# liaochikon/SnowMocap

Measured on AMD Instinct MI355X. Metric: joint-triangulations/sec, higher is better.
Workload: dtype f64; 1 GPU; BASELINE configs[1]: 4 cameras x 1 person x 133 joints x 10000 frames per step per GPU, floor rig, default thresholds; steps cycle a pool of 32 distinct HBM-resident batches; cameras=4, persons=1, joints=133, method=pairwise (reference-exact), io=fp32 in / fp32 out, fp64 math, streams=2, context_overrides=, parallelism=frames sharded x1, no data-path collective

## Files before the change

snowmocap_amd/csrc/snowtri.hip:

```cpp
#include "../../include/snowtri.h"

#include <hip/hip_runtime.h>
#include <hip/hip_ext.h>

#include <algorithm>
#include <atomic>
#include <chrono>
#include <thread>
#include <cmath>
#include <cstdio>
#include <cstdlib>
#include <cstring>
#include <limits>
#include <map>
#include <mutex>
#include <new>
#include <string>
#include <vector>

#include "snowtri_fused.hpp"
#include "snowtri_lean.hpp"
#include "snowtri_cluster.hpp"
#include "snowtri_general.hpp"
#include "snowtri_assoc.hpp"
// ... 2437 lines not shown
    return SNOWTRI_OK;
}

constexpr int kLeanJ = 133;
constexpr int kFusedSingleMaxCams = 4;
constexpr int kLeanTilesPerWave = 4;

template <int C, typename TIn, typename TOut>
std::string lean_kernel_name(const char *kernel) {
    std::vector<std::string> args{std::to_string(C), type_name<TIn>(), std::to_string(kLeanJ)};
    if (sizeof(TOut) == 8) args.push_back("double");
    return kernel_name(kernel, args);
}

template <int C, typename TIn, typename TOut = float>
int launch_fused_lean(snowtri_ctx *ctx, hipStream_t st, int64_t F, const TIn *d_kpts, const int32_t *d_np,
                      const Params &prm, TOut *d_xyzs, TOut *d_ps, int32_t *d_cnt, uint32_t *d_fl) {
    constexpr int kScoreBytes = (int)sizeof(TOut);
    constexpr int NP = C * (C - 1) / 2;
    const int wg_small = ctx->lean_wg_per_cu, tpw = ctx->lean_tiles_per_wave > 0 ? ctx->lean_tiles_per_wave : kLeanTilesPerWave;
    const size_t per_block = general_scratch_bytes(NP, kLeanJ);
    auto kern = k_fused_lean<C, TIn, kLeanJ, TOut>;
    const int64_t W_small = (int64_t)ctx->num_cus * wg_small * kLeanWaves;
    const int64_t seg_max = (int64_t)kLeanTw * kLeanWaves * 512 * ((int64_t)ctx->num_cus * 6);
    LeanUnits<C, TOut> un{};
    if constexpr (LeanUnits<C, TOut>::kUsed) {
        un.lam = prm.dthr;
        un.inv = 1.0 / prm.dthr;
        un.kos = (0.00025 / (double)NP) / prm.dthr;
        for (int q = 0; q < NP; q++)
            for (int i = 0; i < 3; i++)
                un.d[3 * q + i] = (ctx->ht[3 * ctx->hpairs[2 * q + 1] + i] - ctx->ht[3 * ctx->hpairs[2 * q] + i]) * un.inv;
    }
    if (ctx->lean_coop != 0 && F <= (int64_t)ctx->num_cus * wg_small * kCoopMaxFrames) {
        const int grid = (int)std::min<int64_t>(F, (int64_t)ctx->num_cus * wg_small);
        const int base = (int)(F / grid);
        const int64_t rem = F % grid;
        const int nf_max = base + (rem ? 1 : 0);
        const size_t lds = lean_coop_lds_bytes(C, kLeanJ, nf_max, kScoreBytes);
        int rc = ctx->cur->work.ensure(per_block * (size_t)grid);
        if (rc) return rc;
        if (ctx->debug) fprintf(stderr, "k_fused_lean_coop: F %lld grid %d frames per tile %d (+1 for %lld) lds %zu\n", (long long)F, grid, base, (long long)rem, lds);
        rc = launch_kernel(ctx, st, k_fused_lean_coop<C, TIn, kLeanJ, TOut>, dim3(grid), dim3(kBlock), lds, true, F, base, rem, nf_max, ctx->rig(),
                           d_kpts, d_np, prm, un, d_xyzs, d_ps, d_cnt, d_fl, (char *)ctx->cur->work.p, per_block);
        if (rc) return rc;
        static const std::string cname = lean_kernel_name<C, TIn, TOut>("k_fused_lean_coop");
        ctx->last_kernels = cname.c_str();
        return SNOWTRI_OK;
    }
    if (ctx->timing && ctx->timing_attach && F > seg_max) {
        HIP_TRY(hipEventRecord(ctx->ev[0], st));
        HIP_TRY(hipEventRecord(ctx->ev_ring[2 * (ctx->ev_count % kTimingRing)], st));
    }
    for (int64_t s0 = 0; s0 < F; s0 += seg_max) {
        const int64_t Fs = std::min<int64_t>(seg_max, F - s0);
        int64_t W;
        if (Fs <= W_small * kLeanTw) {
            W = std::min<int64_t>(W_small, Fs);
        } else {
            const int64_t tiles0 = (Fs + kLeanTw - 1) / kLeanTw;
            W = std::max<int64_t>(W_small, (tiles0 + tpw - 1) / tpw);
        }
        const size_t scratch_mb = (size_t)ctx->lean_scratch_mb;
        const int64_t grid_cap = std::max<int64_t>((int64_t)ctx->num_cus * 6, (int64_t)((scratch_mb << 20) / per_block));
        const int grid = (int)std::min<int64_t>(grid_cap, (W + kLeanWaves - 1) / kLeanWaves);
        W = (int64_t)grid * kLeanWaves;
        const int64_t tiles_per_wave = (Fs + W * kLeanTw - 1) / (W * kLeanTw);
        const int64_t ntiles = std::min<int64_t>(Fs, W * tiles_per_wave);
// ... 13 lines not shown
            (void)hipOccupancyMaxActiveBlocksPerMultiprocessor(&occ, kern, kBlock, lds);
            fprintf(stderr, "k_fused_lean: F %lld grid %d tiles %lld (%d frames +1 for %lld) lds %zu occupancy/CU %d\n",
                    (long long)Fs, grid, (long long)ntiles, base, (long long)rem, lds, occ);
        }
    }
    static const std::string name = lean_kernel_name<C, TIn, TOut>("k_fused_lean");
    ctx->last_kernels = name.c_str();
    return SNOWTRI_OK;
}

template <typename TIn, typename TOut>
int launch_frame_general(snowtri_ctx *ctx, hipStream_t st, int64_t F, int Pmax, int J, const TIn *d_kpts,
                         const int32_t *d_np, const Params &prm, int Pout, TOut *d_xyzs, TOut *d_ps,
                         int32_t *d_cnt, uint32_t *d_fl) {
    const int64_t Kc = snowtri_num_candidate_slots(ctx->C, Pmax);
    if (Kc > kCondenseMaxN) return SNOWTRI_ERR_BAD_ARG;
    const size_t per_block = std::max<size_t>(256, general_scratch_bytes(Kc, J));
    int64_t grid = std::min<int64_t>(F, (int64_t)ctx->num_cus * 2);
    grid = std::max<int64_t>(1, std::min<int64_t>(grid, (int64_t)(kMaxScratchBytes / per_block)));
    int rc = ctx->cur->work.ensure(per_block * (size_t)grid);
    if (rc) return rc;
    rc = launch_kernel(ctx, st, k_frame_general<TIn, TOut>, dim3((int)grid), dim3(kBlock), condense_lds_bytes((int)Kc), false, F, Pmax, J, (int)Kc,
                       ctx->rig(), d_kpts, d_np, prm, Pout, d_xyzs, d_ps, d_cnt, d_fl, (char *)ctx->cur->work.p, per_block);
    if (rc) return rc;
    static const std::string name = kernel_name("k_frame_general", {type_name<TIn>(), type_name<TOut>()});
    ctx->last_kernels = name.c_str();
    return SNOWTRI_OK;
}

template <int C, typename TIn, typename TOut>
int launch_dlt_coop(snowtri_ctx *ctx, hipStream_t st, int64_t F, const TIn *d_kpts, const int32_t *d_np, const Params &prm, TOut *d_xyzs,
                    TOut *d_ps, int32_t *d_cnt, uint32_t *d_fl) {
    const int64_t resident = (int64_t)ctx->num_cus * kDltCoopWaves;
    const int64_t tiles = std::max<int64_t>((F + kCoopMaxFrames - 1) / kCoopMaxFrames, std::min<int64_t>(F, resident));
    const int base = (int)(F / tiles);
    const int64_t rem = F % tiles;
    const int nf_max = base + (rem ? 1 : 0);
    const size_t lds = dlt_coop_lds_bytes(C, kLeanJ, nf_max, (int)sizeof(TOut));
    int rc = launch_kernel(ctx, st, k_dlt_coop<C, TIn, kLeanJ, TOut>, dim3((unsigned)tiles), dim3(kBlock), lds, true, F, base, rem, nf_max,
                           ctx->rig(), d_kpts, d_np, prm, d_xyzs, d_ps, d_cnt, d_fl);
    if (rc) return rc;
    static const std::string name = kernel_name("k_dlt_coop", {std::to_string(C), type_name<TIn>(), std::to_string(kLeanJ), type_name<TOut>()});
    ctx->last_kernels = name.c_str();
    return SNOWTRI_OK;
}

struct SumsLaunch {
    int threads, lds, per_cu, Jc;
};
SumsLaunch sums_launch_shape(const snowtri_ctx *ctx, int Pmax, int J) {
    const int C = ctx->C, gs = p1_group_size(Pmax);
    const int64_t nitems = (int64_t)ctx->npairs * (Pmax / (gs >= 2 ? kSumsGA : 1)) * (Pmax / gs);
    SumsLaunch L;
    L.threads = ctx->sums_threads > 0 ? ctx->sums_threads : (nitems <= 256 ? 256 : (nitems <= 768 ? 512 : 1024));
    L.threads = L.threads <= 256 ? 256 : (L.threads <= 512 ? 512 : 1024);
    L.lds = ctx->sums_lds_kb > 0 ? ctx->sums_lds_kb * 1024 : (L.threads <= 256 ? 52 * 1024 : (L.threads <= 512 ? 80 * 1024 : 160 * 1024));
    L.lds = std::min(L.lds, 160 * 1024);
    L.per_cu = std::max(1, std::min((160 * 1024) / L.lds, 2048 / L.threads));
    const int pf = L.threads == 256 ? SumsShape<256>::kPrefetch : (L.threads == 512 ? SumsShape<512>::kPrefetch : SumsShape<1024>::kPrefetch);
    L.Jc = sums_chunk_joints(C, Pmax, J, ctx->npairs, L.threads, pf, L.lds);
    return L;
}

struct RecomputeRoute {
    bool can_hand, sumless, sums_kn, post_scores, stream, handover;
    bool split;
    SumsLaunch SL;
// ... 689 lines not shown
```

snowmocap_amd/csrc/snowtri_dlt_lean.hpp:

```cpp
#pragma once
#include "snowtri_lean.hpp"

namespace snowtri {

constexpr int kDltCoopWaves = 3;
__host__ __device__ constexpr size_t dlt_coop_lds_bytes(int C, int JC, int nf_max, int score_bytes = 4) {
    return (((size_t)96 * C + 8 * kDltFrame + (size_t)4 * (lean_coop_items_pad(JC, nf_max) + 128) + (size_t)score_bytes * lean_coop_items_pad(JC, nf_max) +
             (size_t)12 * kCoopMaxFrames + 16) + 15) & ~(size_t)15;
}

template <int C, typename TIn, int JC, typename TOut>
__global__ __launch_bounds__(kBlock, kDltCoopWaves) void k_dlt_coop(int64_t F, int tile_base, int64_t tile_rem, int nf_max, Rig rig,
                                                         const TIn *__restrict__ kpts, const int32_t *__restrict__ n_persons, Params prm,
                                                         TOut *__restrict__ out4, TOut *__restrict__ out_ps, int32_t *__restrict__ out_count,
                                                         uint32_t *__restrict__ out_flags) {
    extern __shared__ __attribute__((aligned(16))) char smem[];
    constexpr unsigned kRec = (unsigned)sizeof(Kp3<TIn>);
    constexpr unsigned kCamStride = (unsigned)JC * kRec;
    constexpr unsigned kOutRec = 4u * (unsigned)sizeof(TOut);
    const int tid = threadIdx.x, lane = tid & 63;
    const int wave = __builtin_amdgcn_readfirstlane(tid >> 6);
    const int items_pad = lean_coop_items_pad(JC, nf_max), ntable = items_pad + 128;
    double *Pl = reinterpret_cast<double *>(smem);
    uint32_t *table = reinterpret_cast<uint32_t *>(Pl + 12 * C + kDltFrame);
    TOut *stash = reinterpret_cast<TOut *>(table + ntable);
    double *favg = reinterpret_cast<double *>(stash + items_pad);
    uint32_t *fmask = reinterpret_cast<uint32_t *>(favg + kCoopMaxFrames);
    const Kp3<TIn> *kp3 = reinterpret_cast<const Kp3<TIn> *>(kpts);
    Kp3<TIn> bufA[C], bufB[C];

    int64_t f0;
    int nf;
    lean_tile_range((int64_t)blockIdx.x, tile_base, tile_rem, f0, nf);
    SNOWTRI_DEV_CHECK(f0 >= 0 && nf >= 1 && nf <= nf_max && nf_max <= kCoopMaxFrames && f0 + nf <= F, 34);
    const int npass_tile = (nf * JC + 63) >> 6;
    const int pos = (wave + 2 * (int)(blockIdx.x & 1u)) & (kLeanWaves - 1);
    const int pq = npass_tile / kLeanWaves, pr = npass_tile - pq * kLeanWaves;
    const int p0 = pos * pq + (pos < pr ? pos : pr), npass = pq + (pos < pr ? 1 : 0);
    const unsigned i0 = (unsigned)p0 * 64u;
    const __amdgpu_buffer_rsrc_t rin = lean_rsrc(kp3 + f0 * (int64_t)(C * JC), (unsigned)(nf * C * JC) * kRec);
    const __amdgpu_buffer_rsrc_t rout = lean_rsrc(reinterpret_cast<char *>(out4) + f0 * (int64_t)JC * kOutRec, (unsigned)(nf * JC) * kOutRec);
    auto fetch = [&](Kp3<TIn>(&dst)[C], unsigned voff) {
#pragma unroll
        for (int c = 0; c < C; c++)
            dst[c] = lean_load_kp3<TIn>(rin, voff + (unsigned)(c & 1) * kCamStride, (unsigned)(c & ~1) * kCamStride);
    };
    auto item_offset = [&](unsigned i) { return (i + (i / (unsigned)JC) * (unsigned)((C - 1) * JC)) * kRec; };
    const double cP = rig.P[tid < 12 * C + kDltFrame ? tid : 0];
    uint32_t cmask = 0xffffu;
    if (n_persons && tid < nf) {
        cmask = 0u;
        for (int c = 0; c < C; c++) cmask |= n_persons[(f0 + tid) * C + c] > 0 ? (1u << c) : 0u;
    }
    constexpr unsigned kNoItem = 0x40000000u;
    fetch(bufA, npass > 0 ? item_offset(i0 + (unsigned)lane) : kNoItem);
    for (unsigned i = (unsigned)tid; i < (unsigned)ntable; i += kBlock) table[i] = item_offset(i);
    if (tid < 12 * C + kDltFrame) Pl[tid] = cP;
    if (tid < kCoopMaxFrames) fmask[tid] = cmask;
    const bool masked = n_persons != nullptr;
    __syncthreads();

    auto solve_store = [&](const Kp3<TIn>(&buf)[C], unsigned out_off, TOut *stash_slot) {
        uint32_t m = 0xffffu;
        if (masked) {
            unsigned o = out_off;
            const unsigned fl = (o / kOutRec) / (unsigned)JC;
            m = fmask[fl < (unsigned)kCoopMaxFrames ? fl : 0u];
        }
        double x, y, z, os;
        asm volatile("" ::: "memory");
        dlt_item<C, TIn>(Pl, buf, m, prm, x, y, z, os);
        if constexpr (sizeof(TOut) == 4) {
            const float osf = (float)os;
            lean_u4 rec;
            rec.x = __float_as_uint((float)x);
            rec.y = __float_as_uint((float)y);
            rec.z = __float_as_uint((float)z);
            rec.w = __float_as_uint(osf);
            __builtin_amdgcn_raw_buffer_store_b128(rec, rout, (int)out_off, 0, kLeanStoreAux);
            *stash_slot = osf;
        } else {
            lean_u4 lo, hi;
            lo.x = (unsigned)__double2loint(x);
            lo.y = (unsigned)__double2hiint(x);
            lo.z = (unsigned)__double2loint(y);
            lo.w = (unsigned)__double2hiint(y);
            hi.x = (unsigned)__double2loint(z);
            hi.y = (unsigned)__double2hiint(z);
            hi.z = (unsigned)__double2loint(os);
            hi.w = (unsigned)__double2hiint(os);
            __builtin_amdgcn_raw_buffer_store_b128(lo, rout, (int)out_off, 0, kLeanStoreAux);
            __builtin_amdgcn_raw_buffer_store_b128(hi, rout, (int)out_off + 16, 0, kLeanStoreAux);
            *stash_slot = os;
        }
    };
    {
        unsigned out_off = (i0 + (unsigned)lane) * kOutRec;
        TOut *sp = stash + i0 + lane;
        const uint32_t *tp = table + i0 + lane;
        for (int k = 0; k < npass; k += 2) {
// ... 32 lines not shown
```

snowmocap_amd/csrc/snowtri_lean.hpp:

```cpp
#pragma once
#include "snowtri_fused.hpp"

namespace snowtri {

#ifndef SNOWTRI_LEAN_ROLLED_WAVES
#define SNOWTRI_LEAN_ROLLED_WAVES 2
#endif
#ifndef SNOWTRI_LEAN_ROLLED_RING
#define SNOWTRI_LEAN_ROLLED_RING 2
#endif
#ifndef SNOWTRI_LEAN_ROLLED_GROUP
#define SNOWTRI_LEAN_ROLLED_GROUP 4
#endif
constexpr int kLeanRolledWaves = SNOWTRI_LEAN_ROLLED_WAVES, kLeanRolledRing = SNOWTRI_LEAN_ROLLED_RING;
constexpr int kLeanRolledGroup = SNOWTRI_LEAN_ROLLED_GROUP;
#ifndef SNOWTRI_LEAN_AUTO_RESIDENT
#define SNOWTRI_LEAN_AUTO_RESIDENT 0
#endif
constexpr bool kLeanAutoResident = SNOWTRI_LEAN_AUTO_RESIDENT;
template <int C, typename TOut = float>
struct LeanShape {
    static constexpr bool kRolled = C >= 6 || (C == 5 && sizeof(TOut) == 8);
    static constexpr int kWaves = kRolled ? kLeanRolledWaves : kFastWaves;
    static constexpr int kRing = kRolled ? kLeanRolledRing : 3;
// ... 44 lines not shown
    if constexpr (sizeof(TIn) == 4) {
        const lean_u3 w = __builtin_amdgcn_raw_buffer_load_b96(r, (int)voff, (int)soff, kLeanLoadAux);
        k.u = __uint_as_float(w.x);
        k.v = __uint_as_float(w.y);
        k.s = __uint_as_float(w.z);
    } else {
        const lean_u4 w = __builtin_amdgcn_raw_buffer_load_b128(r, (int)voff, (int)soff, kLeanLoadAux);
        const lean_u2 z = __builtin_amdgcn_raw_buffer_load_b64(r, (int)voff + 16, (int)soff, kLeanLoadAux);
        k.u = __hiloint2double((int)w.y, (int)w.x);
        k.v = __hiloint2double((int)w.w, (int)w.z);
        k.s = __hiloint2double((int)z.y, (int)z.x);
    }
    return k;
}

__device__ __forceinline__ double uniform_f64(double x) {
    const int lo = __builtin_amdgcn_readfirstlane(__double2loint(x));
    const int hi = __builtin_amdgcn_readfirstlane(__double2hiint(x));
    return __hiloint2double(hi, lo);
}

__device__ __forceinline__ double uniform_lane_f64(double x, int lane) {
    const int lo = __builtin_amdgcn_readlane(__double2loint(x), lane);
    const int hi = __builtin_amdgcn_readlane(__double2hiint(x), lane);
    return __hiloint2double(hi, lo);
}

__device__ __forceinline__ float select_by_mask(float x, unsigned long long mask) {
    float r;
    asm("v_cndmask_b32_e64 %0, 0, %1, %2" : "=v"(r) : "v"(x), "s"(mask));
    return r;
}

template <int NK>
__device__ __forceinline__ void lean_rig_regs_load(double (&Kr)[NK], const double *__restrict__ Mlds) {
    constexpr int C = NK / 12;
#pragma unroll
    for (int i = 0; i < 9 * C + 3; i++) Kr[i] = Mlds[i];
#pragma unroll
    for (int i = 9 * C + 3; i < NK; i++) Kr[i] = Mlds[lean_scaled_at(C) + i - (9 * C + 3)];
#pragma unroll
    for (int i = 0; i < NK; i++) asm volatile("" : "+v"(Kr[i]));
}

template <int C, bool kResident, typename TIn, int NK>
__device__ __forceinline__ bool lean_item(const double *__restrict__ Mlds, const double (&Kr)[NK],
                                          const double (&dS)[3 * (C * (C - 1) / 2)],
                                          const Kp3<TIn> (&cur)[C], float kthr_f32, double kthr, double lam, double kos,
                                          float &ox, float &oy, float &oz, double &os) {
#pragma clang fp contract(off)
    double Mp[9 * C];
    const double *tp;
    if constexpr (kResident) {
        static_assert(NK == 12 * C, "Kr: M[C][9], t_0, t'[1 .. C-1][3]");
#pragma unroll
        for (int i = 0; i < 9 * C; i++) Mp[i] = Kr[i];
        tp = Kr + 9 * C;
    } else {
#pragma unroll
        for (int i = 0; i < 9 * C; i++) Mp[i] = Mlds[i];
        __builtin_amdgcn_sched_barrier(0);
        tp = Mlds + 9 * C;
    }
    double tq[3 * C];
#pragma unroll
    for (int i = 3; i < 3 * C; i++) {
        if constexpr (kResident)
            tq[i] = Kr[9 * C + i];
        else
            tq[i] = dS[i - 3];
    }
    Vec3 h[C], X[C];
    double a[C], alpha[C], beta[C];
    unsigned long long okm[C];
#pragma unroll
    for (int c = 0; c < C; c++) {
        const double u = (double)cur[c].u, v = (double)cur[c].v;
        h[c].x = fma(Mp[9 * c + 0], u, fma(Mp[9 * c + 1], v, Mp[9 * c + 2]));
        h[c].y = fma(Mp[9 * c + 3], u, fma(Mp[9 * c + 4], v, Mp[9 * c + 5]));
        h[c].z = fma(Mp[9 * c + 6], u, fma(Mp[9 * c + 7], v, Mp[9 * c + 8]));
        a[c] = dot3(h[c], h[c]);
        if constexpr (sizeof(TIn) == 4)
            okm[c] = __ballot(!((float)cur[c].s < kthr_f32));
        else
            okm[c] = __ballot(!((double)cur[c].s < kthr));
        if (c >= 1) {
            X[c].x = fma(h[c].y, tq[3 * c + 2], -(h[c].z * tq[3 * c + 1]));
            X[c].y = fma(h[c].z, tq[3 * c + 0], -(h[c].x * tq[3 * c + 2]));
            X[c].z = fma(h[c].x, tq[3 * c + 1], -(h[c].y * tq[3 * c + 0]));
        }
    }
    int q = 0;
#pragma unroll
    for (int mc = 0; mc < C - 1; mc++) {
#pragma unroll
        for (int sc = mc + 1; sc < C; sc++, q++) {
            const Vec3 &hm = h[mc], &hs = h[sc];
            const double dx = mc == 0 ? tq[3 * sc] : dS[3 * q], dy = mc == 0 ? tq[3 * sc + 1] : dS[3 * q + 1],
                         dz = mc == 0 ? tq[3 * sc + 2] : dS[3 * q + 2];
            const double b = dot3(hm, hs);
            const double det = a[mc] * a[sc] - b * b;
            const double e = fma(hm.z, dz, fma(hm.y, dy, hm.x * dx));
            const double g = fma(hs.z, dz, fma(hs.y, dy, hs.x * dx));
// ... 190 lines not shown
    const double cD = rig.pairc[tid < 3 * NP ? 6 * (tid / 3) + tid % 3 : 0];
    const int32_t cP = rig.pairs[tid < 2 * NP ? tid : 0];
    double dS[kRolled ? 1 : 3 * NP];
    constexpr bool kResident = !kRolled && kLeanAutoResident;
    double Kr[kResident ? 12 * C : 1];
    if constexpr (!kRolled) {
#pragma unroll
        for (int i = 0; i < 3 * NP; i++) dS[i] = un.d[i];
    }
    int64_t tile = (int64_t)blockIdx.x * kLeanWaves + wave;
    int64_t f0 = 0;
    int nf = 0;
    if (tile < ntiles) {
        lean_tile_range(tile, tile_base, tile_rem, f0, nf);
        const __amdgpu_buffer_rsrc_t rin = lean_rsrc(kp3 + f0 * (int64_t)(C * JC), (unsigned)(nf * C * JC) * kRec);
        fetch(bufA, rin, voff0);
        if constexpr (kRing >= 3) fetch(bufB, rin, voff1);
    }
    for (unsigned i = (unsigned)tid; i < (unsigned)kTable; i += kBlock)
        table[i] = (i + (i / (unsigned)JC) * (unsigned)((C - 1) * JC)) * kRec;
    for (int i = tid; i < slow_words; i += kBlock) slowbits[i] = 0u;
    if (tid < 9 * C) Mlds[tid] = cM;
    if (tid < 3 * C) Mlds[9 * C + tid] = cT;
    if (tid < 3 * NP) Mlds[12 * C + tid] = cD;
    if constexpr (!kRolled) {
        if (tid < 3 * NP) Mlds[lean_scaled_at(C) + tid] = cD * un.inv;
    }
    int32_t *pairs_lds = reinterpret_cast<int32_t *>(Mlds + 12 * C + 3 * NP);
    if (tid < 2 * NP) pairs_lds[tid] = cP;
    const float kthr_f32 = prm.kthr_f32;
    const double kthr = prm.kthr, dthr2 = prm.dthr2;
    const double ctol2_lo = prm.ctol < 0.0 ? -1.0 : prm.ctol * prm.ctol * (1.0 - 1e-12);
    __syncthreads();
    if constexpr (kResident) lean_rig_regs_load(Kr, Mlds);

    for (int ord = 0; tile < ntiles; tile += wstride, ord++) {
        SNOWTRI_DEV_CHECK(f0 >= 0 && nf >= 1 && nf <= kLeanTw && f0 + nf <= F, 1);
        SNOWTRI_DEV_CHECK((ord * kLeanWaves + wave + 1) << kLeanSlowShift <= slow_words * 32, 2);
        const __amdgpu_buffer_rsrc_t rin = lean_rsrc(kp3 + f0 * (int64_t)(C * JC), (unsigned)(nf * C * JC) * kRec);
        const __amdgpu_buffer_rsrc_t rout =
            lean_rsrc(reinterpret_cast<char *>(out4) + f0 * (int64_t)JC * kOutRec, (unsigned)(nf * JC) * kOutRec);
        const unsigned last = (unsigned)(nf * JC - 1);
        const int npass = (nf * JC + 63) >> 6;
        const unsigned slow_base = (unsigned)((ord * kLeanWaves + wave) << kLeanSlowShift);
        constexpr int kCheckFrames = 64 / NP;
        constexpr int kCheckPre = kRolled ? 0 : 2;
        Kp3<TIn> ckm[kCheckPre ? kCheckPre : 1], cks[kCheckPre ? kCheckPre : 1];
#pragma unroll
        for (int pass = 0; pass < kCheckPre; pass++) {
            const int wl = lane / NP, qq = lane - wl * NP, w = pass * kCheckFrames + wl;
            const bool live = wl < kCheckFrames && w < nf;
            const Kp3<TIn> *p = kp3 + (f0 + (live ? w : 0)) * (int64_t)(C * JC) + prm.center;
            ckm[pass] = p[pairs_lds[2 * qq] * JC];
            cks[pass] = p[pairs_lds[2 * qq + 1] * JC];
        }

        auto solve_store = [&](const Kp3<TIn>(&buf)[C], unsigned out_off, TOut *stash_slot) {
            const bool bad = lean_solve_store<C, kResident, TIn, TOut>(Mlds, Kr, dS, buf, kthr_f32, kthr, dthr2, un.lam, un.kos, rout, out_off, stash_slot);
            if (__ballot(bad)) {
                unsigned o = out_off;
                asm volatile("" : "+v"(o));
                const unsigned i = o / kOutRec;
                const unsigned bit = slow_base + i / (unsigned)JC;
                if (bad && i <= last) atomicOr(&slowbits[bit >> 5], 1u << (bit & 31u));
            }
        };
        unsigned out_off = (unsigned)lane * kOutRec;
// ... 54 lines not shown
                km = ckm[pass];
                ks = cks[pass];
            } else {
                const Kp3<TIn> *p = kp3 + (f0_cur + (live ? w : 0)) * (int64_t)(C * JC) + prm.center;
                km = p[mc * JC];
                ks = p[sc * JC];
            }
            const bool far = lean_centre_far<C, TIn>(Mlds, mc, sc, qq, lane, km, ks, ctol2_lo);
            if (live && far) {
                const unsigned bit = slow_base + (unsigned)w;
                atomicOr(&slowbits[bit >> 5], 1u << (bit & 31u));
            }
        }
        __builtin_amdgcn_fence(__ATOMIC_ACQ_REL, "wavefront");
        {
            constexpr int G = 4;
            const int w = lane / G, sub = lane & (G - 1);
            const bool live = w < nf_cur;
            const int64_t f = f0_cur + (live ? w : 0);
            double sum = 0.0;
            if (live) sum = lean_row_partial<JC, TOut>(stash + w * JC, sub);
            int not_one = 0;
            if (n_persons && live)
                for (int c = sub; c < C; c += G) not_one |= n_persons[f * C + c] != 1;
#pragma unroll
            for (int off = G / 2; off > 0; off >>= 1) {
                sum += __shfl_xor(sum, off, 64);
                not_one |= __shfl_xor(not_one, off, 64);
            }
            if (live && sub == 0) {
                const double avg = sum / (double)JC;
                const unsigned bit = slow_base + (unsigned)w;
                const bool slow = ((slowbits[bit >> 5] >> (bit & 31u)) & 1u) != 0u || !(avg >= prm.score_tol) ||
                                  fabs(avg - prm.score_tol) < 1e-6 * fabs(prm.score_tol) || not_one != 0;
                if (slow) {
                    atomicOr(&slowbits[bit >> 5], 1u << (bit & 31u));
                } else {
                    out_count[f] = 1;
                    if (out_ps) out_ps[f] = (TOut)avg;
                    if (out_flags) out_flags[f] = kFlagFast;
                }
            }
        }
        __builtin_amdgcn_fence(__ATOMIC_ACQ_REL, "wavefront");
    }

    __syncthreads();
    unsigned any = 0u;
    for (int i = lane; i < slow_words; i += 64) any |= slowbits[i];
    if (__ballot(any != 0u) == 0ull) return;
    {
        const PackedWriter<TOut> wr{out4, out_ps};
        double *slab = reinterpret_cast<double *>(scratch + (size_t)blockIdx.x * scratch_per_block);
        for (int wd = 0; wd < slow_words; wd++) {
            uint32_t m = slowbits[wd];
            __syncthreads();
            while (m) {
                const int bpos = __ffs((int)m) - 1;
                m &= m - 1u;
                const unsigned bit = (unsigned)(wd * 32 + bpos);
                const unsigned slot = bit >> kLeanSlowShift;
                const int64_t t = (int64_t)blockIdx.x * kLeanWaves + (slot % kLeanWaves) + (int64_t)(slot / kLeanWaves) * wstride;
                int64_t tf0;
                int tnf;
                lean_tile_range(t, tile_base, tile_rem, tf0, tnf);
                general_frame<TIn>(tf0 + (bit & ((1u << kLeanSlowShift) - 1u)), 1, JC, NP, rig, kpts, n_persons, prm, 1, wr,
                                   out_count, out_flags, slab, smem);
            }
        }
    }
}

constexpr int kCoopMaxFrames = 32;
__host__ __device__ constexpr int lean_coop_items_pad(int JC, int nf_max) { return (nf_max * JC + 63) / 64 * 64; }
__host__ __device__ constexpr size_t lean_coop_lds_bytes(int C, int JC, int nf_max, int score_bytes = 4) {
    return (((size_t)8 * lean_const_doubles(C) + (size_t)score_bytes * lean_coop_items_pad(JC, nf_max) + (size_t)8 * kCoopMaxFrames + 16) + 15) & ~(size_t)15;
}

template <int C, typename TIn, int JC, typename TOut = float>
__global__ __launch_bounds__(kBlock, (LeanShape<C, TOut>::kWaves)) void k_fused_lean_coop(
    int64_t F, int tile_base, int64_t tile_rem, int nf_max, Rig rig, const TIn *__restrict__ kpts, const int32_t *__restrict__ n_persons,
    Params prm, LeanUnits<C, TOut> un, TOut *__restrict__ out4, TOut *__restrict__ out_ps, int32_t *__restrict__ out_count,
    uint32_t *__restrict__ out_flags, char *scratch, size_t scratch_per_block) {
    extern __shared__ __attribute__((aligned(16))) char smem[];
    constexpr int NP = C * (C - 1) / 2;
    constexpr int kConstDoubles = lean_const_doubles(C);
    constexpr unsigned kRec = (unsigned)sizeof(Kp3<TIn>);
    constexpr unsigned kCamStride = (unsigned)JC * kRec;
    const int tid = threadIdx.x, lane = tid & 63;
    const int wave = __builtin_amdgcn_readfirstlane(tid >> 6);
    const int items_pad = lean_coop_items_pad(JC, nf_max);
    double *Mlds = reinterpret_cast<double *>(smem);
    TOut *stash = reinterpret_cast<TOut *>(Mlds + kConstDoubles);
    double *favg = reinterpret_cast<double *>(stash + items_pad);
    uint32_t *slowbits = reinterpret_cast<uint32_t *>(favg + kCoopMaxFrames);
    const Kp3<TIn> *kp3 = reinterpret_cast<const Kp3<TIn> *>(kpts);
    constexpr bool kRolled = LeanShape<C, TOut>::kRolled;
    constexpr unsigned kOutRec = 4u * (unsigned)sizeof(TOut);
    static_assert(sizeof(TOut) == 4 || kRolled, "float64 outputs: the rolled item only");
    constexpr int kRing = (kRolled && sizeof(TIn) == 8 && C >= 8) ? 1 : LeanShape<C, TOut>::kRing;
    Kp3<TIn> bufA[C], bufB[kRing >= 2 ? C : 1], bufC[kRing >= 3 ? C : 1];

#ifdef SNOWTRI_LEAN_TRACE
    unsigned long long *trace = reinterpret_cast<unsigned long long *>(scratch + (size_t)blockIdx.x * scratch_per_block) + 8 * (threadIdx.x >> 6);
#define SNOWTRI_STAMP(i) do { if ((threadIdx.x & 63) == 0) trace[i] = __builtin_amdgcn_s_memrealtime(); } while (0)
#else
#define SNOWTRI_STAMP(i) ((void)0)
#endif
    SNOWTRI_STAMP(0);
#ifdef SNOWTRI_LEAN_TRACE
    if ((threadIdx.x & 63) == 0) {
        unsigned hw, xcc;
        asm volatile("s_getreg_b32 %0, hwreg(HW_REG_HW_ID)" : "=s"(hw));
        asm volatile("s_getreg_b32 %0, hwreg(HW_REG_XCC_ID)" : "=s"(xcc));
        trace[7] = ((unsigned long long)xcc << 32) | hw;
    }
#endif
    int64_t f0;
    int nf;
    lean_tile_range((int64_t)blockIdx.x, tile_base, tile_rem, f0, nf);
    SNOWTRI_DEV_CHECK(f0 >= 0 && nf >= 1 && nf <= nf_max && nf_max <= kCoopMaxFrames && f0 + nf <= F, 3);
    const int npass_tile = (nf * JC + 63) >> 6;
    const int pos = (wave + 2 * (int)(blockIdx.x & 1u)) & (kLeanWaves - 1);
    const int pq = npass_tile / kLeanWaves, pr = npass_tile - pq * kLeanWaves;
    const int p0 = pos * pq + (pos < pr ? pos : pr), npass = pq + (pos < pr ? 1 : 0);
    const unsigned i0 = (unsigned)p0 * 64u;
    const __amdgpu_buffer_rsrc_t rin = lean_rsrc(kp3 + f0 * (int64_t)(C * JC), (unsigned)(nf * C * JC) * kRec);
    const __amdgpu_buffer_rsrc_t rout = lean_rsrc(reinterpret_cast<char *>(out4) + f0 * (int64_t)JC * kOutRec, (unsigned)(nf * JC) * kOutRec);
    const unsigned last = (unsigned)(nf * JC - 1);
    auto fetch = [&](Kp3<TIn>(&dst)[C], unsigned voff) {
#pragma unroll
        for (int c = 0; c < C; c++)
            dst[c] = lean_load_kp3<TIn>(rin, voff + (unsigned)(c & 1) * kCamStride, (unsigned)(c & ~1) * kCamStride);
    };
    static_assert(JC > 64, "one frame boundary per pass of 64 joints");
    constexpr unsigned kNoItem = 0x40000000u;
    constexpr unsigned kFrameSkip = (unsigned)((C - 1) * JC) * kRec;
    unsigned sj = i0 % (unsigned)JC, sbase = (i0 + (i0 / (unsigned)JC) * (unsigned)((C - 1) * JC)) * kRec;
    const unsigned lane_off = (unsigned)lane * kRec;
    auto next_offset = [&](bool own) {
        const unsigned o = lane_off + (own ? sbase : kNoItem) + ((unsigned)lane >= (unsigned)JC - sj ? kFrameSkip : 0u);
        sj += 64u;
        sbase += 64u * kRec;
        if (sj >= (unsigned)JC) {
            sj -= (unsigned)JC;
            sbase += kFrameSkip;
        }
        return o;
    };
    const double cM = rig.M[tid < 9 * C ? tid : 0], cT = rig.t[tid < 3 * C ? tid : 0];
    const double cD = rig.pairc[tid < 3 * NP ? 6 * (tid / 3) + tid % 3 : 0];
    const int32_t cP = rig.pairs[tid < 2 * NP ? tid : 0];
    double dS[kRolled ? 1 : 3 * NP];
    constexpr bool kResident = !kRolled && C == 4 && sizeof(TIn) == 4;
    double Kr[kResident ? 12 * C : 1];
    if constexpr (!kRolled) {
#pragma unroll
        for (int i = 0; i < 3 * NP; i++) dS[i] = un.d[i];
    }
    fetch(bufA, next_offset(npass > 0));
    if constexpr (kRing >= 3) fetch(bufB, next_offset(npass > 1));
    constexpr int kCheckFrames = 64 / NP;
    const int ncheck = (nf + kCheckFrames - 1) / kCheckFrames;
    Kp3<TIn> ckm, cks;
    int32_t *pairs_lds = reinterpret_cast<int32_t *>(Mlds + 12 * C + 3 * NP);
    if (tid == 0) slowbits[0] = 0u;
    if (tid < 9 * C) Mlds[tid] = cM;
    if (tid < 3 * C) Mlds[9 * C + tid] = cT;
    if (tid < 3 * NP) Mlds[12 * C + tid] = cD;
    if constexpr (!kRolled) {
        if (tid < 3 * NP) Mlds[lean_scaled_at(C) + tid] = cD * un.inv;
    }
    if (tid < 2 * NP) pairs_lds[tid] = cP;
    const float kthr_f32 = prm.kthr_f32;
    const double kthr = prm.kthr, dthr2 = prm.dthr2;
    const double ctol2_lo = prm.ctol < 0.0 ? -1.0 : prm.ctol * prm.ctol * (1.0 - 1e-12);
    SNOWTRI_STAMP(1);
    __syncthreads();
    SNOWTRI_STAMP(2);
    if constexpr (kResident) lean_rig_regs_load(Kr, Mlds);
    {
        const int wl = lane / NP, qq = lane - wl * NP, w = pos * kCheckFrames + wl;
        const bool live = pos < ncheck && wl < kCheckFrames && w < nf;
        const Kp3<TIn> *p = kp3 + (f0 + (live ? w : 0)) * (int64_t)(C * JC) + prm.center;
        ckm = p[pairs_lds[2 * qq] * JC];
        cks = p[pairs_lds[2 * qq + 1] * JC];
    }

    auto solve_store = [&](const Kp3<TIn>(&buf)[C], unsigned out_off, TOut *stash_slot) {
        const bool bad = lean_solve_store<C, kResident, TIn, TOut>(Mlds, Kr, dS, buf, kthr_f32, kthr, dthr2, un.lam, un.kos, rout, out_off, stash_slot);
        if (__ballot(bad)) {
            unsigned o = out_off;
            asm volatile("" : "+v"(o));
            const unsigned i = o / kOutRec;
            if (bad && i <= last) atomicOr(&slowbits[0], 1u << (i / (unsigned)JC));
        }
    };
    {
        unsigned out_off = (i0 + (unsigned)lane) * kOutRec;
        TOut *sp = stash + i0 + lane;
        if constexpr (kRing >= 3) {
            for (int k = 0; k < npass; k += 3) {
                fetch(bufC, next_offset(k + 2 < npass));
                solve_store(bufA, out_off, sp);
                fetch(bufA, next_offset(k + 3 < npass));
                if (k + 1 < npass) solve_store(bufB, out_off + 64u * kOutRec, sp + 64);
                fetch(bufB, next_offset(k + 4 < npass));
                if (k + 2 < npass) solve_store(bufC, out_off + 128u * kOutRec, sp + 128);
                out_off += 192u * kOutRec;
                sp += 192;
            }
        } else if constexpr (kRing == 2) {
            for (int k = 0; k < npass; k += 2) {
                fetch(bufB, next_offset(k + 1 < npass));
                solve_store(bufA, out_off, sp);
                fetch(bufA, next_offset(k + 2 < npass));
                if (k + 1 < npass) solve_store(bufB, out_off + 64u * kOutRec, sp + 64);
                out_off += 128u * kOutRec;
                sp += 128;
            }
        } else {
            for (int k = 0; k < npass; k++) {
                solve_store(bufA, out_off, sp);
                fetch(bufA, next_offset(k + 1 < npass));
                out_off += 64u * kOutRec;
                sp += 64;
            }
        }
    }
    SNOWTRI_STAMP(3);
    __syncthreads();
    SNOWTRI_STAMP(4);

    for (int pass = pos; pass < ncheck; pass += kLeanWaves) {
        const int wl = lane / NP, qq = lane - wl * NP, w = pass * kCheckFrames + wl;
        const bool live = wl < kCheckFrames && w < nf;
        const int mc = pairs_lds[2 * qq], sc = pairs_lds[2 * qq + 1];
        Kp3<TIn> km = ckm, ks = cks;
        if (pass != pos) {
            const Kp3<TIn> *p = kp3 + (f0 + (live ? w : 0)) * (int64_t)(C * JC) + prm.center;
            km = p[mc * JC];
            ks = p[sc * JC];
        }
        const bool far = lean_centre_far<C, TIn>(Mlds, mc, sc, qq, lane, km, ks, ctol2_lo);
        if (live && far) atomicOr(&slowbits[0], 1u << w);
    }
    {
        constexpr int G = 4;
        const int nmean = (nf + 64 / G - 1) / (64 / G);
        for (int pass = (pos - ncheck) & (kLeanWaves - 1); pass < nmean; pass += kLeanWaves) {
            const int w = pass * (64 / G) + lane / G, sub = lane & (G - 1);
            const bool live = w < nf;
            const int64_t f = f0 + (live ? w : 0);
            double sum = 0.0;
            if (live) sum = lean_row_partial<JC, TOut>(stash + w * JC, sub);
            int not_one = 0;
            if (n_persons && live)
                for (int c = sub; c < C; c += G) not_one |= n_persons[f * C + c] != 1;
#pragma unroll
            for (int off = G / 2; off > 0; off >>= 1) {
                sum += __shfl_xor(sum, off, 64);
                not_one |= __shfl_xor(not_one, off, 64);
            }
            if (live && sub == 0) {
                const double avg = sum / (double)JC;
                favg[w] = avg;
                if (!(avg >= prm.score_tol) || fabs(avg - prm.score_tol) < 1e-6 * fabs(prm.score_tol) || not_one != 0)
                    atomicOr(&slowbits[0], 1u << w);
            }
        }
    }
    SNOWTRI_STAMP(5);
    __syncthreads();
    const uint32_t slow = slowbits[0];
    if (wave == 0 && lane < nf && !((slow >> lane) & 1u)) {
        const int64_t f = f0 + lane;
        out_count[f] = 1;
        if (out_ps) out_ps[f] = (TOut)favg[lane];
        if (out_flags) out_flags[f] = kFlagFast;
    }
    SNOWTRI_STAMP(6);
    if (slow == 0u) return;
    {
        const PackedWriter<TOut> wr{out4, out_ps};
        double *slab = reinterpret_cast<double *>(scratch + (size_t)blockIdx.x * scratch_per_block);
        uint32_t m = slow;
        __syncthreads();
        while (m) {
            const int bpos = __ffs((int)m) - 1;
            m &= m - 1u;
            general_frame<TIn>(f0 + bpos, 1, JC, NP, rig, kpts, n_persons, prm, 1, wr, out_count, out_flags, slab, smem);
        }
    }
}

}
```

Measured before the change: 69.03 billion joints/s.

## Widen coop lean tiles, scalarize input streaming, and drop per-item bad checks

Splits the coop frame limit into a 64-frame cap, used only with an off-by-default overlap mode, and a 32-frame lone cap, with slow-frame bitmasks widened to 64 bits. Adds compile-time trims that are on by default: a scalar-offset buffer resource per fetch to cut per-lane address math, keeping only t_0 resident in registers instead of all translations, and skipping the per-item ballot/atomic for bad solves in the resident path. To keep fallbacks correct without the per-item check, the frame-level test now also marks non-finite score sums as slow. The DLT coop kernel gets its own 32-frame constant. These trims aim to cut VGPR pressure and instruction count in the hot loop, at the cost of relying on the score-sum check to catch bad items.

```diff
diff --git a/snowmocap_amd/csrc/snowtri.hip b/snowmocap_amd/csrc/snowtri.hip
--- a/snowmocap_amd/csrc/snowtri.hip
+++ b/snowmocap_amd/csrc/snowtri.hip
@@ -2493,8 +2493,10 @@
             for (int i = 0; i < 3; i++)
                 un.d[3 * q + i] = (ctx->ht[3 * ctx->hpairs[2 * q + 1] + i] - ctx->ht[3 * ctx->hpairs[2 * q] + i]) * un.inv;
     }
-    if (ctx->lean_coop != 0 && F <= (int64_t)ctx->num_cus * wg_small * kCoopMaxFrames) {
-        const int grid = (int)std::min<int64_t>(F, (int64_t)ctx->num_cus * wg_small);
+    const bool beside = kCoopOverlapWide && ctx->overlap >= 2 && ctx->cur != &ctx->sets[0] && F <= (int64_t)ctx->num_cus * kCoopMaxFrames;
+    const int wg_coop = beside ? 1 : wg_small;
+    if (ctx->lean_coop != 0 && F <= (int64_t)ctx->num_cus * wg_coop * (beside ? kCoopMaxFrames : kCoopLoneFrames)) {
+        const int grid = (int)std::min<int64_t>(F, (int64_t)ctx->num_cus * wg_coop);
         const int base = (int)(F / grid);
         const int64_t rem = F % grid;
         const int nf_max = base + (rem ? 1 : 0);
@@ -2574,7 +2576,7 @@
 int launch_dlt_coop(snowtri_ctx *ctx, hipStream_t st, int64_t F, const TIn *d_kpts, const int32_t *d_np, const Params &prm, TOut *d_xyzs,
                     TOut *d_ps, int32_t *d_cnt, uint32_t *d_fl) {
     const int64_t resident = (int64_t)ctx->num_cus * kDltCoopWaves;
-    const int64_t tiles = std::max<int64_t>((F + kCoopMaxFrames - 1) / kCoopMaxFrames, std::min<int64_t>(F, resident));
+    const int64_t tiles = std::max<int64_t>((F + kDltCoopMaxFrames - 1) / kDltCoopMaxFrames, std::min<int64_t>(F, resident));
     const int base = (int)(F / tiles);
     const int64_t rem = F % tiles;
     const int nf_max = base + (rem ? 1 : 0);
diff --git a/snowmocap_amd/csrc/snowtri_dlt_lean.hpp b/snowmocap_amd/csrc/snowtri_dlt_lean.hpp
--- a/snowmocap_amd/csrc/snowtri_dlt_lean.hpp
+++ b/snowmocap_amd/csrc/snowtri_dlt_lean.hpp
@@ -3,10 +3,11 @@
 
 namespace snowtri {
 
+constexpr int kDltCoopMaxFrames = 32;
 constexpr int kDltCoopWaves = 3;
 __host__ __device__ constexpr size_t dlt_coop_lds_bytes(int C, int JC, int nf_max, int score_bytes = 4) {
     return (((size_t)96 * C + 8 * kDltFrame + (size_t)4 * (lean_coop_items_pad(JC, nf_max) + 128) + (size_t)score_bytes * lean_coop_items_pad(JC, nf_max) +
-             (size_t)12 * kCoopMaxFrames + 16) + 15) & ~(size_t)15;
+             (size_t)12 * kDltCoopMaxFrames + 16) + 15) & ~(size_t)15;
 }
 
 template <int C, typename TIn, int JC, typename TOut>
@@ -25,14 +26,14 @@
     uint32_t *table = reinterpret_cast<uint32_t *>(Pl + 12 * C + kDltFrame);
     TOut *stash = reinterpret_cast<TOut *>(table + ntable);
     double *favg = reinterpret_cast<double *>(stash + items_pad);
-    uint32_t *fmask = reinterpret_cast<uint32_t *>(favg + kCoopMaxFrames);
+    uint32_t *fmask = reinterpret_cast<uint32_t *>(favg + kDltCoopMaxFrames);
     const Kp3<TIn> *kp3 = reinterpret_cast<const Kp3<TIn> *>(kpts);
     Kp3<TIn> bufA[C], bufB[C];
 
     int64_t f0;
     int nf;
     lean_tile_range((int64_t)blockIdx.x, tile_base, tile_rem, f0, nf);
-    SNOWTRI_DEV_CHECK(f0 >= 0 && nf >= 1 && nf <= nf_max && nf_max <= kCoopMaxFrames && f0 + nf <= F, 34);
+    SNOWTRI_DEV_CHECK(f0 >= 0 && nf >= 1 && nf <= nf_max && nf_max <= kDltCoopMaxFrames && f0 + nf <= F, 34);
     const int npass_tile = (nf * JC + 63) >> 6;
     const int pos = (wave + 2 * (int)(blockIdx.x & 1u)) & (kLeanWaves - 1);
     const int pq = npass_tile / kLeanWaves, pr = npass_tile - pq * kLeanWaves;
@@ -56,7 +57,7 @@
     fetch(bufA, npass > 0 ? item_offset(i0 + (unsigned)lane) : kNoItem);
     for (unsigned i = (unsigned)tid; i < (unsigned)ntable; i += kBlock) table[i] = item_offset(i);
     if (tid < 12 * C + kDltFrame) Pl[tid] = cP;
-    if (tid < kCoopMaxFrames) fmask[tid] = cmask;
+    if (tid < kDltCoopMaxFrames) fmask[tid] = cmask;
     const bool masked = n_persons != nullptr;
     __syncthreads();
 
@@ -65,7 +66,7 @@
         if (masked) {
             unsigned o = out_off;
             const unsigned fl = (o / kOutRec) / (unsigned)JC;
-            m = fmask[fl < (unsigned)kCoopMaxFrames ? fl : 0u];
+            m = fmask[fl < (unsigned)kDltCoopMaxFrames ? fl : 0u];
         }
         double x, y, z, os;
         asm volatile("" ::: "memory");
diff --git a/snowmocap_amd/csrc/snowtri_lean.hpp b/snowmocap_amd/csrc/snowtri_lean.hpp
--- a/snowmocap_amd/csrc/snowtri_lean.hpp
+++ b/snowmocap_amd/csrc/snowtri_lean.hpp
@@ -100,9 +100,9 @@
     return r;
 }
 
-template <int NK>
+template <int C, int NK>
 __device__ __forceinline__ void lean_rig_regs_load(double (&Kr)[NK], const double *__restrict__ Mlds) {
-    constexpr int C = NK / 12;
+    static_assert(NK == 12 * C || NK == 9 * C + 3, "Kr: M[C][9], t_0 and, at 12 C, t'[1 .. C-1][3]");
 #pragma unroll
     for (int i = 0; i < 9 * C + 3; i++) Kr[i] = Mlds[i];
 #pragma unroll
@@ -119,8 +119,9 @@
 #pragma clang fp contract(off)
     double Mp[9 * C];
     const double *tp;
+    constexpr bool kScalarT = !kResident || NK == 9 * C + 3;
     if constexpr (kResident) {
-        static_assert(NK == 12 * C, "Kr: M[C][9], t_0, t'[1 .. C-1][3]");
+        static_assert(NK == 12 * C || NK == 9 * C + 3, "Kr: M[C][9], t_0 and, at 12 C, t'[1 .. C-1][3]");
 #pragma unroll
         for (int i = 0; i < 9 * C; i++) Mp[i] = Kr[i];
         tp = Kr + 9 * C;
@@ -133,10 +134,10 @@
     double tq[3 * C];
 #pragma unroll
     for (int i = 3; i < 3 * C; i++) {
-        if constexpr (kResident)
+        if constexpr (kScalarT)
+            tq[i] = dS[i - 3];
+        else
             tq[i] = Kr[9 * C + i];
-        else
-            tq[i] = dS[i - 3];
     }
     Vec3 h[C], X[C];
     double a[C], alpha[C], beta[C];
@@ -393,7 +394,7 @@
     const double kthr = prm.kthr, dthr2 = prm.dthr2;
     const double ctol2_lo = prm.ctol < 0.0 ? -1.0 : prm.ctol * prm.ctol * (1.0 - 1e-12);
     __syncthreads();
-    if constexpr (kResident) lean_rig_regs_load(Kr, Mlds);
+    if constexpr (kResident) lean_rig_regs_load<C>(Kr, Mlds);
 
     for (int ord = 0; tile < ntiles; tile += wstride, ord++) {
         SNOWTRI_DEV_CHECK(f0 >= 0 && nf >= 1 && nf <= kLeanTw && f0 + nf <= F, 1);
@@ -514,7 +515,8 @@
                 const double avg = sum / (double)JC;
                 const unsigned bit = slow_base + (unsigned)w;
                 const bool slow = ((slowbits[bit >> 5] >> (bit & 31u)) & 1u) != 0u || !(avg >= prm.score_tol) ||
-                                  fabs(avg - prm.score_tol) < 1e-6 * fabs(prm.score_tol) || not_one != 0;
+                                  fabs(avg - prm.score_tol) < 1e-6 * fabs(prm.score_tol) || not_one != 0 ||
+                                  !(fabs(sum) < INFINITY);
                 if (slow) {
                     atomicOr(&slowbits[bit >> 5], 1u << (bit & 31u));
                 } else {
@@ -553,7 +555,17 @@
     }
 }
 
-constexpr int kCoopMaxFrames = 32;
+constexpr int kCoopMaxFrames = 64;
+constexpr int kCoopLoneFrames = 32;
+#ifndef SNOWTRI_COOP_OVERLAP_WIDE
+#define SNOWTRI_COOP_OVERLAP_WIDE 0
+#endif
+constexpr bool kCoopOverlapWide = SNOWTRI_COOP_OVERLAP_WIDE;
+#ifndef SNOWTRI_COOP_TRIMS
+#define SNOWTRI_COOP_TRIMS 7
+#endif
+constexpr bool kCoopNoItemCheck = (SNOWTRI_COOP_TRIMS & 1) != 0, kCoopScalarStream = (SNOWTRI_COOP_TRIMS & 2) != 0,
+               kCoopScalarT = (SNOWTRI_COOP_TRIMS & 4) != 0;
 __host__ __device__ constexpr int lean_coop_items_pad(int JC, int nf_max) { return (nf_max * JC + 63) / 64 * 64; }
 __host__ __device__ constexpr size_t lean_coop_lds_bytes(int C, int JC, int nf_max, int score_bytes = 4) {
     return (((size_t)8 * lean_const_doubles(C) + (size_t)score_bytes * lean_coop_items_pad(JC, nf_max) + (size_t)8 * kCoopMaxFrames + 16) + 15) & ~(size_t)15;
@@ -576,6 +588,8 @@
     TOut *stash = reinterpret_cast<TOut *>(Mlds + kConstDoubles);
     double *favg = reinterpret_cast<double *>(stash + items_pad);
     uint32_t *slowbits = reinterpret_cast<uint32_t *>(favg + kCoopMaxFrames);
+    static_assert(kCoopMaxFrames <= 64, "slow frames: two 32-bit words; count / score / flags: one lane of wave 0 per frame");
+    auto mark_slow = [&](unsigned w) { atomicOr(&slowbits[w >> 5], 1u << (w & 31u)); };
     const Kp3<TIn> *kp3 = reinterpret_cast<const Kp3<TIn> *>(kpts);
     constexpr bool kRolled = LeanShape<C, TOut>::kRolled;
     constexpr unsigned kOutRec = 4u * (unsigned)sizeof(TOut);
@@ -610,6 +624,7 @@
     const __amdgpu_buffer_rsrc_t rin = lean_rsrc(kp3 + f0 * (int64_t)(C * JC), (unsigned)(nf * C * JC) * kRec);
     const __amdgpu_buffer_rsrc_t rout = lean_rsrc(reinterpret_cast<char *>(out4) + f0 * (int64_t)JC * kOutRec, (unsigned)(nf * JC) * kOutRec);
     const unsigned last = (unsigned)(nf * JC - 1);
+    (void)last;
     auto fetch = [&](Kp3<TIn>(&dst)[C], unsigned voff) {
 #pragma unroll
         for (int c = 0; c < C; c++)
@@ -620,33 +635,54 @@
     constexpr unsigned kFrameSkip = (unsigned)((C - 1) * JC) * kRec;
     unsigned sj = i0 % (unsigned)JC, sbase = (i0 + (i0 / (unsigned)JC) * (unsigned)((C - 1) * JC)) * kRec;
     const unsigned lane_off = (unsigned)lane * kRec;
-    auto next_offset = [&](bool own) {
-        const unsigned o = lane_off + (own ? sbase : kNoItem) + ((unsigned)lane >= (unsigned)JC - sj ? kFrameSkip : 0u);
+    auto step_stream = [&]() {
         sj += 64u;
         sbase += 64u * kRec;
         if (sj >= (unsigned)JC) {
             sj -= (unsigned)JC;
             sbase += kFrameSkip;
         }
+    };
+    auto next_offset = [&](bool own) {
+        const unsigned o = lane_off + (own ? sbase : kNoItem) + ((unsigned)lane >= (unsigned)JC - sj ? kFrameSkip : 0u);
+        step_stream();
         return o;
+    };
+    const char *const tile_in = reinterpret_cast<const char *>(kp3 + f0 * (int64_t)(C * JC));
+    const unsigned tile_bytes = (unsigned)(nf * C * JC) * kRec, lane_off_skip = lane_off + kFrameSkip;
+    auto fetch_next = [&](Kp3<TIn>(&dst)[C], bool own) {
+        if constexpr (kCoopScalarStream) {
+            const unsigned before = (unsigned)JC - sj;
+            const unsigned long long behind = before < 64u ? ~0ull << before : 0ull;
+            SNOWTRI_DEV_CHECK(!own || (sj < (unsigned)JC && sbase < tile_bytes), 4);
+            unsigned voff;
+            asm("v_cndmask_b32_e64 %0, %1, %2, %3" : "=v"(voff) : "v"(lane_off), "v"(lane_off_skip), "s"(behind));
+            const __amdgpu_buffer_rsrc_t r = lean_rsrc(tile_in + sbase, own ? tile_bytes - sbase : 0u);
+            step_stream();
+#pragma unroll
+            for (int c = 0; c < C; c++)
+                dst[c] = lean_load_kp3<TIn>(r, voff + (unsigned)(c & 1) * kCamStride, (unsigned)(c & ~1) * kCamStride);
+        } else {
+            fetch(dst, next_offset(own));
+        }
     };
     const double cM = rig.M[tid < 9 * C ? tid : 0], cT = rig.t[tid < 3 * C ? tid : 0];
     const double cD = rig.pairc[tid < 3 * NP ? 6 * (tid / 3) + tid % 3 : 0];
     const int32_t cP = rig.pairs[tid < 2 * NP ? tid : 0];
     double dS[kRolled ? 1 : 3 * NP];
     constexpr bool kResident = !kRolled && C == 4 && sizeof(TIn) == 4;
-    double Kr[kResident ? 12 * C : 1];
+    double Kr[kResident ? (kCoopScalarT ? 9 * C + 3 : 12 * C) : 1];
     if constexpr (!kRolled) {
 #pragma unroll
         for (int i = 0; i < 3 * NP; i++) dS[i] = un.d[i];
     }
-    fetch(bufA, next_offset(npass > 0));
-    if constexpr (kRing >= 3) fetch(bufB, next_offset(npass > 1));
+    fetch_next(bufA, npass > 0);
+    if constexpr (kRing >= 3) fetch_next(bufB, npass > 1);
     constexpr int kCheckFrames = 64 / NP;
     const int ncheck = (nf + kCheckFrames - 1) / kCheckFrames;
     Kp3<TIn> ckm, cks;
     int32_t *pairs_lds = reinterpret_cast<int32_t *>(Mlds + 12 * C + 3 * NP);
-    if (tid == 0) slowbits[0] = 0u;
+    if (tid < 2) slowbits[tid] = 0u;
     if (tid < 9 * C) Mlds[tid] = cM;
     if (tid < 3 * C) Mlds[9 * C + tid] = cT;
     if (tid < 3 * NP) Mlds[12 * C + tid] = cD;
@@ -660,7 +696,7 @@
     SNOWTRI_STAMP(1);
     __syncthreads();
     SNOWTRI_STAMP(2);
-    if constexpr (kResident) lean_rig_regs_load(Kr, Mlds);
+    if constexpr (kResident) lean_rig_regs_load<C>(Kr, Mlds);
     {
         const int wl = lane / NP, qq = lane - wl * NP, w = pos * kCheckFrames + wl;
         const bool live = pos < ncheck && wl < kCheckFrames && w < nf;
@@ -671,11 +707,13 @@
 
     auto solve_store = [&](const Kp3<TIn>(&buf)[C], unsigned out_off, TOut *stash_slot) {
         const bool bad = lean_solve_store<C, kResident, TIn, TOut>(Mlds, Kr, dS, buf, kthr_f32, kthr, dthr2, un.lam, un.kos, rout, out_off, stash_slot);
-        if (__ballot(bad)) {
-            unsigned o = out_off;
-            asm volatile("" : "+v"(o));
-            const unsigned i = o / kOutRec;
-            if (bad && i <= last) atomicOr(&slowbits[0], 1u << (i / (unsigned)JC));
+        if constexpr (!(kResident && kCoopNoItemCheck)) {
+            if (__ballot(bad)) {
+                unsigned o = out_off;
+                asm volatile("" : "+v"(o));
+                const unsigned i = o / kOutRec;
+                if (bad && i <= last) mark_slow(i / (unsigned)JC);
+            }
         }
     };
     {
@@ -683,20 +721,20 @@
         TOut *sp = stash + i0 + lane;
         if constexpr (kRing >= 3) {
             for (int k = 0; k < npass; k += 3) {
-                fetch(bufC, next_offset(k + 2 < npass));
+                fetch_next(bufC, k + 2 < npass);
                 solve_store(bufA, out_off, sp);
-                fetch(bufA, next_offset(k + 3 < npass));
+                fetch_next(bufA, k + 3 < npass);
                 if (k + 1 < npass) solve_store(bufB, out_off + 64u * kOutRec, sp + 64);
-                fetch(bufB, next_offset(k + 4 < npass));
+                fetch_next(bufB, k + 4 < npass);
                 if (k + 2 < npass) solve_store(bufC, out_off + 128u * kOutRec, sp + 128);
                 out_off += 192u * kOutRec;
                 sp += 192;
             }
         } else if constexpr (kRing == 2) {
             for (int k = 0; k < npass; k += 2) {
-                fetch(bufB, next_offset(k + 1 < npass));
+                fetch_next(bufB, k + 1 < npass);
                 solve_store(bufA, out_off, sp);
-                fetch(bufA, next_offset(k + 2 < npass));
+                fetch_next(bufA, k + 2 < npass);
                 if (k + 1 < npass) solve_store(bufB, out_off + 64u * kOutRec, sp + 64);
                 out_off += 128u * kOutRec;
                 sp += 128;
@@ -704,7 +742,7 @@
         } else {
             for (int k = 0; k < npass; k++) {
                 solve_store(bufA, out_off, sp);
-                fetch(bufA, next_offset(k + 1 < npass));
+                fetch_next(bufA, k + 1 < npass);
                 out_off += 64u * kOutRec;
                 sp += 64;
             }
@@ -725,7 +763,7 @@
             ks = p[sc * JC];
         }
         const bool far = lean_centre_far<C, TIn>(Mlds, mc, sc, qq, lane, km, ks, ctol2_lo);
-        if (live && far) atomicOr(&slowbits[0], 1u << w);
+        if (live && far) mark_slow((unsigned)w);
     }
     {
         constexpr int G = 4;
@@ -747,14 +785,14 @@
             if (live && sub == 0) {
                 const double avg = sum / (double)JC;
                 favg[w] = avg;
-                if (!(avg >= prm.score_tol) || fabs(avg - prm.score_tol) < 1e-6 * fabs(prm.score_tol) || not_one != 0)
-                    atomicOr(&slowbits[0], 1u << w);
+                if (!(avg >= prm.score_tol) || fabs(avg - prm.score_tol) < 1e-6 * fabs(prm.score_tol) || not_one != 0 || !(fabs(sum) < INFINITY))
+                    mark_slow((unsigned)w);
             }
         }
     }
     SNOWTRI_STAMP(5);
     __syncthreads();
-    const uint32_t slow = slowbits[0];
+    const uint64_t slow = (uint64_t)slowbits[0] | ((uint64_t)slowbits[1] << 32);
     if (wave == 0 && lane < nf && !((slow >> lane) & 1u)) {
         const int64_t f = f0 + lane;
         out_count[f] = 1;
@@ -766,10 +804,10 @@
     {
         const PackedWriter<TOut> wr{out4, out_ps};
         double *slab = reinterpret_cast<double *>(scratch + (size_t)blockIdx.x * scratch_per_block);
-        uint32_t m = slow;
+        uint64_t m = slow;
         __syncthreads();
         while (m) {
-            const int bpos = __ffs((int)m) - 1;
+            const int bpos = __ffsll((unsigned long long)m) - 1;
             m &= m - 1u;
             general_frame<TIn>(f0 + bpos, 1, JC, NP, rig, kpts, n_persons, prm, 1, wr, out_count, out_flags, slab, smem);
         }
```

New measurement: 69.60 billion joints/s, median of 6. About the same (+0.8%).
